# david-wb/tiny-diffusion

Measured on AMD Instinct MI355X. Metric: train images/s (q_sample+fwd+MSE+bwd+allreduce+Adam), MNIST 28x28 UNet fp32; 1000-step sample latency in `sample`, higher is better.
Workload: dtype f32; 1 GPU; diffusion.py unconditional MNIST 28x28 UNet, fp32, train step, batch 256/GPU (BASELINE.json configs[1]); global_batch=256, per_gpu_batch=256, parallelism=dp1

## Files before the change

include/tdx.h:

```cpp
#ifndef TDX_H
#define TDX_H

#include <stddef.h>
#include <stdint.h>

#ifdef __cplusplus
extern "C" {
#endif

#define TDX_VERSION 400

#define TDX_E_BADARG (-1)
#define TDX_E_SHAPE (-2)
#define TDX_E_WORKSPACE (-3)
#define TDX_E_STATE (-4)

typedef void* tdx_stream_t;

int tdx_version(void);
const char* tdx_error_string(int code);


int tdx_q_sample(const float* x0, const float* noise, const int64_t* t,
                 const float* sqrt_ac, const float* sqrt_1mac, float* x_t,
// ... 51 lines not shown

#define TDX_CONV_IN_BNRELU 1
#define TDX_CONV_OUT_BNRELU 2
#define TDX_CONV_OUT_STATS 4

size_t tdx_edge_conv_wgrad_scratch_floats(int B, int H, int W);
int tdx_initial_conv_forward(const float* x, const float* w, const float* bias, float* out, int B, int H, int W,
                             int cin, int cout, tdx_stream_t stream);
int tdx_initial_conv_backward(const float* x, const float* g_out, float* dw, float* db, float* scratch, int B,
                              int H, int W, int cin, int cout, tdx_stream_t stream);
int tdx_initial_conv_input_grad(const float* g_out, const float* w, float* g_x, int B, int H, int W, int cin,
                                int cout, tdx_stream_t stream);
int tdx_final_conv_forward(const float* in, const float* w, const float* bias, float* out, int B, int H, int W,
                           int cout, tdx_stream_t stream);
int tdx_final_conv_backward(const float* in, const float* g_out, const float* w, float* g_in, float* dw, float* db,
                            float* scratch, int B, int H, int W, int cout, tdx_stream_t stream);

int tdx_conv3x3_fwd(const float* in, const float* wpk, const float* bias, float* out,
                    int B, int H, int W, int cin, int cout, int flags,
                    const float* in_scale, const float* in_shift,
                    const float* out_scale, const float* out_shift,
                    float* stats_partial, tdx_stream_t stream);
int tdx_conv3x3_fwd_splitk(const float* in, const float* wpk, const float* bias, float* out,
                           int B, int H, int W, int cin, int cout, int flags,
                           const float* in_scale, const float* in_shift,
                           const float* out_scale, const float* out_shift,
                           float* scratch, size_t scratch_floats, tdx_stream_t stream);
size_t tdx_conv3x3_splitk_scratch_floats(int B, int H, int W, int cin, int cout);
int tdx_conv3x3_wino_ok(int B, int H, int W, int cin, int cout);
int tdx_pack_conv3x3_wino(const float* w_oihw, float* u_fwd, float* u_dgrad, int cout, int cin, tdx_stream_t stream);
int tdx_conv3x3_fwd_wino(const float* in, const float* u, const float* bias, float* out, int B, int H, int W,
                         int cin, int cout, int flags, const float* out_scale, const float* out_shift,
                         float* stats_partial, tdx_stream_t stream);
int tdx_conv3x3_fwd_wino_infer(const float* in, const float* u, const float* bias, float* out, int B, int H, int W,
                               int cin, int cout, const float* out_scale, const float* out_shift, float* scratch,
                               size_t scratch_floats, tdx_stream_t stream);
int tdx_conv3x3_train_algo(int B, int H, int W, int cin, int cout, int role);
int tdx_conv3x3_infer_algo(int B, int H, int W, int cin, int cout);
int tdx_conv3x3_wgrad_wino_splits(int B, int H, int W, int cin, int cout);
int tdx_conv3x3_wgrad_wino(const float* in, const float* dy, float* dw_slabs, int B, int H, int W, int cin, int cout,
                           tdx_stream_t stream);
int tdx_conv3x3_wino_stat_tiles(int B, int H, int W);
int tdx_conv3x3_wino_stat_tile_rows(int B, int H, int W);
int tdx_pack_conv3x3_tiled(const float* w_oihw, float* w_tiled, int cout, int cin, tdx_stream_t stream);
int tdx_conv3x3_fwd_infer(const float* in, const float* w_tiled, const float* bias, float* out, int B, int H, int W,
                          int cin, int cout, const float* out_scale, const float* out_shift, float* scratch,
                          size_t scratch_floats, tdx_stream_t stream);
size_t tdx_conv3x3_infer_scratch_floats(int B, int H, int W, int cin, int cout);
int tdx_conv3x3_fwd_train(const float* in, const float* wpk, const float* bias, float* out, int B, int H, int W,
                          int cin, int cout, int flags, float* stats_partial, float* scratch,
                          size_t scratch_floats, tdx_stream_t stream);
size_t tdx_conv3x3_train_scratch_floats(int B, int H, int W, int cin, int cout);
int tdx_conv3x3_stat_tiles(int B, int H, int W, int cin, int cout);
int tdx_conv3x3_stat_tile_rows(int B, int H, int W, int cin, int cout);
int tdx_conv3x3_shape_ok(int B, int H, int W, int cin, int cout);
int tdx_conv3x3_tile_shape(int B, int H, int W, int cin, int cout, int role);

int tdx_conv3x3_dgrad(const float* dy, const float* w_dgrad, float* dx, int B, int H, int W,
                      int cin, int cout, tdx_stream_t stream);

int tdx_conv3x3_wgrad_splits(int B, int H, int W, int cin, int cout);
int tdx_conv3x3_wgrad(const float* in, const float* dy, float* dw_slabs,
                      int B, int H, int W, int cin, int cout, int flags,
                      const float* in_scale, const float* in_shift, tdx_stream_t stream);
int tdx_conv3x3_wgrad_reduce(const float* dw_slabs, float* dw_oihw, int splits, int cout, int cin,
                             tdx_stream_t stream);
// ... 178 lines not shown
```

tiny_diffusion_amd/_lib.py:

```python
from __future__ import annotations

import ctypes as C
import os

import torch

from . import _build

_c_float_p = C.c_void_p
_c_i64_p = C.c_void_p
_ptr = C.c_void_p


class TdxError(RuntimeError):
    pass


def _load():
    path = _build.LIB
    if not os.path.exists(path):
        if os.environ.get("TDX_NO_AUTOBUILD"):
            raise TdxError(
                f"{path} not found: build it with `python -m tiny_diffusion_amd._build` "
                "(there is no CPU fallback for the HIP path)"
# ... 16 lines not shown


lib = _load()

_SIGS = {
    "tdx_version": (C.c_int, []),
    "tdx_error_string": (C.c_char_p, [C.c_int]),
    "tdx_q_sample": (C.c_int, [_ptr, _ptr, _ptr, _ptr, _ptr, _ptr, C.c_int, C.c_int, _ptr]),
    "tdx_q_sample_philox": (C.c_int, [_ptr, _ptr, _ptr, _ptr, _ptr, _ptr, C.c_int, C.c_int,
                                      C.c_uint64, C.c_uint64, _ptr]),
    "tdx_p_sample_step": (C.c_int, [_ptr, _ptr, _ptr, _ptr, _ptr, _ptr, C.c_int64, _ptr]),
    "tdx_p_sample_step_philox": (C.c_int, [_ptr, _ptr, _ptr, _ptr, _ptr, C.c_int64, C.c_uint64, _ptr]),
    "tdx_u8_gather_normalize": (C.c_int, [_ptr, _ptr, _ptr, C.c_int, C.c_int, C.c_float, C.c_float, _ptr]),
    "tdx_mse_loss": (C.c_int, [_ptr, _ptr, _ptr, _ptr, C.c_float, C.c_int64, _ptr]),
    "tdx_mse_scratch_bytes": (C.c_size_t, []),
    "tdx_mse_loss_grad": (C.c_int, [_ptr, _ptr, _ptr, _ptr, C.c_float, C.c_int64, _ptr, _ptr]),
    "tdx_adam_step": (C.c_int, [_ptr, _ptr, _ptr, _ptr, C.c_int64, C.c_float, C.c_float, C.c_float,
                                C.c_float, C.c_int, C.c_float, _ptr]),
    "tdx_adam_clip_scratch_bytes": (C.c_size_t, []),
    "tdx_adam_step_clip": (C.c_int, [_ptr, _ptr, _ptr, _ptr, C.c_int64, C.c_float, C.c_float, C.c_float, C.c_float,
                                     C.c_int, C.c_float, C.c_float, _ptr, _ptr, _ptr]),
    "tdx_edge_conv_wgrad_scratch_floats": (C.c_size_t, [C.c_int] * 3),
    "tdx_initial_conv_forward": (C.c_int, [_ptr, _ptr, _ptr, _ptr, C.c_int, C.c_int, C.c_int, C.c_int, C.c_int, _ptr]),
    "tdx_initial_conv_backward": (C.c_int, [_ptr, _ptr, _ptr, _ptr, _ptr, C.c_int, C.c_int, C.c_int, C.c_int, C.c_int,
                                            _ptr]),
    "tdx_final_conv_forward": (C.c_int, [_ptr, _ptr, _ptr, _ptr, C.c_int, C.c_int, C.c_int, C.c_int, _ptr]),
    "tdx_final_conv_backward": (C.c_int, [_ptr, _ptr, _ptr, _ptr, _ptr, _ptr, _ptr, C.c_int, C.c_int, C.c_int, C.c_int,
                                          _ptr]),
    "tdx_pack_conv3x3": (C.c_int, [_ptr, _ptr, _ptr, C.c_int, C.c_int, _ptr]),
    "tdx_conv3x3_wino_ok": (C.c_int, [C.c_int] * 5),
    "tdx_pack_conv3x3_wino": (C.c_int, [_ptr, _ptr, _ptr, C.c_int, C.c_int, _ptr]),
    "tdx_conv3x3_fwd_wino": (C.c_int, [_ptr, _ptr, _ptr, _ptr, C.c_int, C.c_int, C.c_int, C.c_int, C.c_int, C.c_int, _ptr,
                                       _ptr, _ptr, _ptr]),
    "tdx_conv3x3_fwd_wino_infer": (C.c_int, [_ptr, _ptr, _ptr, _ptr, C.c_int, C.c_int, C.c_int, C.c_int, C.c_int, _ptr, _ptr,
                                             _ptr, C.c_size_t, _ptr]),
    "tdx_conv3x3_train_algo": (C.c_int, [C.c_int] * 6),
    "tdx_conv3x3_infer_algo": (C.c_int, [C.c_int] * 5),
    "tdx_conv3x3_wgrad_wino_splits": (C.c_int, [C.c_int] * 5),
    "tdx_conv3x3_wgrad_wino": (C.c_int, [_ptr, _ptr, _ptr, C.c_int, C.c_int, C.c_int, C.c_int, C.c_int, _ptr]),
    "tdx_conv3x3_wino_stat_tiles": (C.c_int, [C.c_int] * 3),
    "tdx_conv3x3_wino_stat_tile_rows": (C.c_int, [C.c_int] * 3),
    "tdx_pack_conv3x3_tiled": (C.c_int, [_ptr, _ptr, C.c_int, C.c_int, _ptr]),
    "tdx_conv3x3_fwd_infer": (C.c_int, [_ptr, _ptr, _ptr, _ptr, C.c_int, C.c_int, C.c_int, C.c_int, C.c_int, _ptr, _ptr,
                                        _ptr, C.c_size_t, _ptr]),
    "tdx_conv3x3_infer_scratch_floats": (C.c_size_t, [C.c_int] * 5),
    "tdx_conv3x3_fwd": (C.c_int, [_ptr, _ptr, _ptr, _ptr, C.c_int, C.c_int, C.c_int, C.c_int, C.c_int,
                                  C.c_int, _ptr, _ptr, _ptr, _ptr, _ptr, _ptr]),
    "tdx_conv3x3_fwd_splitk": (C.c_int, [_ptr, _ptr, _ptr, _ptr, C.c_int, C.c_int, C.c_int, C.c_int, C.c_int,
                                         C.c_int, _ptr, _ptr, _ptr, _ptr, _ptr, C.c_size_t, _ptr]),
    "tdx_conv3x3_splitk_scratch_floats": (C.c_size_t, [C.c_int] * 5),
    "tdx_conv3x3_fwd_train": (C.c_int, [_ptr, _ptr, _ptr, _ptr, C.c_int, C.c_int, C.c_int, C.c_int, C.c_int, C.c_int,
                                        _ptr, _ptr, C.c_size_t, _ptr]),
    "tdx_conv3x3_train_scratch_floats": (C.c_size_t, [C.c_int] * 5),
    "tdx_conv3x3_stat_tiles": (C.c_int, [C.c_int] * 5),
    "tdx_conv3x3_stat_tile_rows": (C.c_int, [C.c_int] * 5),
    "tdx_conv3x3_wgrad_splits": (C.c_int, [C.c_int] * 5),
    "tdx_diag_conv_occupancy": (C.c_int, [C.c_int]),
    "tdx_conv3x3_wgrad_splits_bf16": (C.c_int, [C.c_int] * 5),
    "tdx_conv3x3_fwd_bf16_io": (C.c_int, [_ptr] * 4 + [C.c_int] * 6 + [_ptr] * 5 + [C.c_int, _ptr]),
    "tdx_conv3x3_wgrad_bf16_io": (C.c_int, [_ptr] * 3 + [C.c_int] * 6 + [_ptr] * 2 + [C.c_int, _ptr]),
    "tdx_conv3x3_shape_ok": (C.c_int, [C.c_int] * 5),
    "tdx_conv3x3_tile_shape": (C.c_int, [C.c_int] * 6),
    "tdx_conv3x3_wgrad": (C.c_int, [_ptr, _ptr, _ptr, C.c_int, C.c_int, C.c_int, C.c_int, C.c_int,
                                    C.c_int, _ptr, _ptr, _ptr]),
    "tdx_conv3x3_wgrad_reduce": (C.c_int, [_ptr, _ptr, C.c_int, C.c_int, C.c_int, _ptr]),
    "tdx_bn_finalize": (C.c_int, [_ptr, C.c_int, C.c_int, C.c_int64, C.c_int, _ptr, _ptr, _ptr, _ptr, _ptr,
# ... 126 lines not shown
```

tiny_diffusion_amd/csrc/conv3x3.hip:

```cpp
#include "internal.h"
#include <cstring>
#include <type_traits>

#define BK 32
#define BKP 36

#include "conv_shared.h"

template <int BM, int BN, bool IN_BN, int EPI>
__global__ void __launch_bounds__(256)
conv3x3_igemm_kernel(ConvArgs a) {
  constexpr int WGM = 2, WGN = 2;
  constexpr int WTM = BM / WGM, WTN = BN / WGN;
  constexpr int TM = WTM / 32, TN = WTN / 32;
  constexpr int AI = BM / 32, BI = BN / 32;
  static_assert(TM >= 1 && TN >= 1, "wave tile must hold a 32x32 MFMA tile");

  extern __shared__ __attribute__((aligned(16))) float smem[];
  float* As = smem;
  float* Bs = smem + 2 * BM * BKP;

  const int tid = threadIdx.x;
  const int lane = tid & 63, wave = tid >> 6;
  const int l31 = lane & 31, half = lane >> 5;
// ... 764 lines not shown
  if (!strcmp(key, "sample_fuse")) { g_tdx_sample_fuse = value & 7; return 0; }
  if (!strcmp(key, "sample_defer_max")) { g_tdx_sample_defer_max = value; return 0; }
  if (!strcmp(key, "sample_tables")) { g_tdx_sample_tables = value != 0; return 0; }
  if (!strcmp(key, "sample_halves")) { g_tdx_sample_halves = value != 0; return 0; }
  if (!strcmp(key, "sample_halves_min")) { g_tdx_sample_halves_min = value > 2 ? value : 2; return 0; }
  if (!strcmp(key, "bnbwd_fused")) { g_tdx_bnbwd_fused = value & 7; return 0; }
  if (!strcmp(key, "conv_hybrid")) { g_conv_hybrid = value != 0; return 0; }
  if (!strcmp(key, "splitk_fused")) { g_splitk_fused = value != 0; return 0; }
  if (!strcmp(key, "splitk_train")) { g_splitk_train = value != 0; return 0; }
  if (!strcmp(key, "splitk_train_t64")) { g_splitk_train_t64 = value > 0 ? value : 1024; return 0; }
  if (!strcmp(key, "splitk_train_target")) { g_splitk_train_target = value > 0 ? value : 1536; return 0; }
  if (!strcmp(key, "splitk_train_any")) { g_splitk_train_any = value != 0; return 0; }
  if (!strcmp(key, "time_proj_early")) { g_tdx_time_proj_early = value != 0; return 0; }
  if (!strcmp(key, "time_stage_diag")) { g_tdx_time_stage = value == 6 ? 6 : 14; return 0; }
  if (!strcmp(key, "time_l1_impl")) { g_tdx_time_l1_impl = value; return 0; }
  if (!strcmp(key, "input_copy")) { g_tdx_input_copy = value; return 0; }
  if (!strcmp(key, "conv_dbg")) { g_conv_dbg = value; return 0; }
  if (!strcmp(key, "bf16_materialize")) { g_tdx_bf16_materialize = value ? 1 : 0; return 0; }
  if (!strcmp(key, "bf16_thin")) { g_tdx_bf16_thin = value < 0 ? 0 : value; return 0; }
  if (!strcmp(key, "bf16_ring")) { g_tdx_bf16_ring = value ? 1 : 0; return 0; }
  if (!strcmp(key, "bf16_wgrad9")) { g_tdx_wgrad9 = value ? 1 : 0; return 0; }
  if (!strcmp(key, "bf16_wgrad_swz")) { g_tdx_wgrad_bf16s = value ? 1 : 0; return 0; }
  if (!strcmp(key, "conv_stamp")) { g_conv_stamp = value; g_tdx_probe_stamp = value; return 0; }
  if (!strcmp(key, "wgrad_small")) { g_wgrad_small = value; return 0; }
  if (!strcmp(key, "wino")) { g_tdx_wino = value != 0; return 0; }
  if (!strcmp(key, "wino_infer")) { g_tdx_wino_infer = value != 0; return 0; }
  if (!strcmp(key, "wino_infer_min_units")) { g_tdx_wino_infer_min_units = value >= 0 ? value : 700; return 0; }
  if (!strcmp(key, "wino_infer_ovh")) { g_wino_infer_ovh = value >= 0 ? value : 2; return 0; }
  if (!strcmp(key, "wino_infer_red")) { g_wino_infer_red = value >= 0 ? value : 3; return 0; }
  if (!strcmp(key, "wino_wgrad")) { g_tdx_wino_wgrad = value != 0; return 0; }
  if (!strcmp(key, "wino_wgrad_min_tiles")) { g_tdx_wino_wgrad_min_tiles = value > 0 ? value : 1024; return 0; }
  if (!strcmp(key, "wino_wgrad_target")) { g_tdx_wino_wgrad_target = value > 0 ? value : 512; return 0; }
  if (!strcmp(key, "wino_min_wgs")) { g_tdx_wino_min_wgs = value > 0 ? value : 1; return 0; }
  if (!strcmp(key, "wino_rows")) { g_tdx_wino_rows = value != 0; return 0; }
  if (!strcmp(key, "wino_rows_min_stages")) { g_tdx_wino_rows_min_stages = value > 0 ? value : 16; return 0; }
  if (!strcmp(key, "infer_ring")) { g_tdx_infer_ring = value != 0; return 0; }
  if (!strcmp(key, "infer_stages")) { g_infer_stages = value == 3 ? 3 : 4; return 0; }
  if (!strcmp(key, "infer_splits")) { g_infer_splits = value > 0 ? value : 0; return 0; }
  if (!strcmp(key, "infer_ovh")) { g_infer_ovh = value >= 0 ? value : 4; return 0; }
  if (!strcmp(key, "infer_red")) { g_infer_red = value >= 0 ? value : 12; return 0; }
  if (!strcmp(key, "infer_cus")) { g_tdx_infer_cus = value > 0 && value <= 256 ? value : 256; return 0; }
  if (!strcmp(key, "wgrad9_wgs")) { g_wgrad9_wgs = value > 0 ? value : 0; return 0; }
  if (!strcmp(key, "wgrad_plan")) { g_wgrad_plan = value; return 0; }
  if (!strcmp(key, "wgrad_rounds")) { g_wgrad_rounds = value; return 0; }
  if (!strcmp(key, "conv_dma")) { g_conv_dma = value; return 0; }
  if (!strcmp(key, "wgrad_target")) { g_wgrad_target = value > 0 ? value : 2048; return 0; }
  if (!strcmp(key, "wgrad_target_big")) { g_wgrad_target_big = value > 0 ? value : 0; return 0; }
  return TDX_E_BADARG;
}

static TileCfg pick_tile(int64_t M, int cout) {
  const TileCfg cands[3] = {{128, 128}, {128, 64}, {64, 64}};
  if (g_force_tile >= 1 && g_force_tile <= 3 && cout % cands[g_force_tile - 1].bn == 0)
    return cands[g_force_tile - 1];
  for (int i = 0; i < 3; ++i) {
    if (cout % cands[i].bn) continue;
    if (i == 2) return cands[i];
    const int64_t tiles = ((M + cands[i].bm - 1) / cands[i].bm) * (cout / cands[i].bn);
    if (tiles < g_min_tiles) continue;
    const int64_t rounds = (tiles + 255) / 256;
    if ((double)(rounds * 256) <= 1.035 * (double)tiles) return cands[i];
  }
  return cands[2];
}

template <int BM, int BN>
// ... 1179 lines not shown
```

tiny_diffusion_amd/csrc/conv3x3_wino.hip:

```cpp
#include "internal.h"
#include "conv_shared.h"

extern unsigned* g_tdx_diag_buffer;
extern size_t g_tdx_diag_bytes;
extern int g_tdx_probe_stamp;

constexpr int WT = 64;
constexpr int WN = 64;
constexpr int WK = 8;
constexpr int A_ST = 16 * WT * WK;
constexpr int B_ST = 16 * WN * WK;
constexpr int STAGE = A_ST + B_ST;

struct WinoArgs {
  const float* in;
  const float* u;
  const float* bias;
  float* out;
  const float* out_scale;
  const float* out_shift;
  float* stats;
  int B, H, W, Cin, Cout, th, tw, NT, tilesN, M;
  float rcp_tpi, rcp_tw;
  int per;
  int compact;
  unsigned long long* stamps;
};

constexpr int OLD = 68;
constexpr int TAB_OFF = 2 * STAGE;
typedef unsigned u32x4 __attribute__((ext_vector_type(4)));

template <int EPI, int XH = -1>
__device__ __forceinline__ void wino_epilogue(const WinoArgs& a, float* out, const float* bias, f32x16 (&acc)[16], float* smem,
                                              int tblk, int n0, int wm, int wn, int l31, int half, int tid,
                                              const f32x4* xin = nullptr) {
#if defined(__HIP_DEVICE_COMPILE__)
  const unsigned* tab = reinterpret_cast<const unsigned*>(smem + TAB_OFF);
  const int cl = wn * 32 + l31, col = n0 + cl;
  const float bv = bias ? bias[col] : 0.f;
  float osc = 1.f, osh = 0.f;
  if (EPI == EPI_BNRELU) { osc = a.out_scale[col]; osh = a.out_shift[col]; }
  float csum = 0.f, cnt = 0.f;
  float* ot = smem;
  f32x4 pv[8];
#pragma unroll
  for (int r = 0; r < 16; ++r) {
    if (XH >= 0 && (r & 3) == 0) {
#pragma unroll
      for (int p = 0; p < 8; ++p) pv[p] = xin[(p * 4 + (r >> 2)) * 64];
    }
    auto M = [&](int p) { return XH >= 0 && (p >> 3) != XH ? pv[p & 7][r & 3] : acc[p][r]; };
    float s0[4], s1[4];
#pragma unroll
    for (int nu = 0; nu < 4; ++nu) {
      s0[nu] = M(0 + nu) + M(4 + nu) + M(8 + nu);
      s1[nu] = M(4 + nu) - M(8 + nu) - M(12 + nu);
    }
    float y[4] = {s0[0] + s0[1] + s0[2], s0[1] - s0[2] - s0[3], s1[0] + s1[1] + s1[2], s1[1] - s1[2] - s1[3]};
    const int tl = wm * 32 + (r & 3) + 8 * (r >> 2) + 4 * half;
    const unsigned m = tab[2 * tl + 1];
#pragma unroll
    for (int q = 0; q < 4; ++q) {
      float val = y[q] + bv;
      if (EPI == EPI_BNRELU) val = fmaxf(fmaf(val, osc, osh), 0.f);
      const bool ok = (m >> q) & 1u;
      if (XH < 0) ot[(tl * 4 + q) * OLD + cl] = val;
      csum += ok ? val : 0.f;
      cnt += ok ? 1.f : 0.f;
      y[q] = ok ? val : 0.f;
    }
    acc[0][r] = y[0]; acc[1][r] = y[1]; acc[4][r] = y[2]; acc[5][r] = y[3];
    acc[2][r] = (m & 1u) ? 1.f : 0.f;
    acc[3][r] = (m & 2u) ? 1.f : 0.f;
    acc[6][r] = (m & 4u) ? 1.f : 0.f;
    acc[7][r] = (m & 8u) ? 1.f : 0.f;
  }
  if (XH >= 0) {
    __syncthreads();
#pragma unroll
    for (int r = 0; r < 16; ++r) {
      const int tl = wm * 32 + (r & 3) + 8 * (r >> 2) + 4 * half;
      ot[(tl * 4 + 0) * OLD + cl] = acc[0][r]; ot[(tl * 4 + 1) * OLD + cl] = acc[1][r];
      ot[(tl * 4 + 2) * OLD + cl] = acc[4][r]; ot[(tl * 4 + 3) * OLD + cl] = acc[5][r];
    }
  }
  __syncthreads();
  {
    const auto rsrc_out = __builtin_amdgcn_make_buffer_rsrc(out, 0, (int)((int64_t)a.M * a.Cout * 4), 0x00020000);
    const int c4 = (tid & 15) * 4, q = (tid >> 4) & 3;
    const unsigned qoff = (unsigned)((((q >> 1) * a.W + (q & 1)) * a.Cout + n0 + c4) * 4);
    const uint2* tab2 = reinterpret_cast<const uint2*>(tab);
    const float* src = ot + (tid >> 4) * OLD + c4;
#pragma unroll
    for (int i = 0; i < 16; ++i) {
      const uint2 e = tab2[4 * i + (tid >> 6)];
      const unsigned off = ((e.y >> q) & 1u) ? e.x + qoff : 0x80000000u;
      const f32x4 v = *reinterpret_cast<const f32x4*>(src + i * 16 * OLD);
      __builtin_amdgcn_raw_buffer_store_b128(__builtin_bit_cast(u32x4, v), rsrc_out, off, 0, 0);
    }
  }
  if (EPI == EPI_STATS) {
    float* red = smem + 256 * OLD;
    const float s = csum + __shfl_xor(csum, 32, 64);
    const float n = cnt + __shfl_xor(cnt, 32, 64);
    if (half == 0) { red[wm * 64 + cl] = s; red[128 + wm * 64 + cl] = n; }
    __syncthreads();
    if (tid < 64) {
      const float ts = red[tid] + red[64 + tid];
      const float tn = red[128 + tid] + red[192 + tid];
      red[256 + tid] = tn > 0.f ? ts / tn : 0.f;
      a.stats[((size_t)tblk * 2 + 0) * a.Cout + n0 + tid] = ts;
    }
    __syncthreads();
    const float mean = red[256 + cl];
    float q = 0.f;
#pragma unroll
    for (int r = 0; r < 16; ++r) {
      const float d0 = acc[0][r] - mean, d1 = acc[1][r] - mean, d2 = acc[4][r] - mean, d3 = acc[5][r] - mean;
      q = fmaf(d0 * acc[2][r], d0, q); q = fmaf(d1 * acc[3][r], d1, q);
      q = fmaf(d2 * acc[6][r], d2, q); q = fmaf(d3 * acc[7][r], d3, q);
    }
    q += __shfl_xor(q, 32, 64);
    __syncthreads();
    if (half == 0) red[wm * 64 + cl] = q;
    __syncthreads();
    if (tid < 64) a.stats[((size_t)tblk * 2 + 1) * a.Cout + n0 + tid] = red[tid] + red[64 + tid];
  }
#endif
}

#if defined(__HIP_DEVICE_COMPILE__)
// ... 333 lines not shown
    gg[3][c] = g[6 + c];
  }
#pragma unroll
  for (int r = 0; r < 4; ++r) {
    U[r * 4 + 0] = gg[r][0];
    U[r * 4 + 1] = 0.5f * (gg[r][0] + gg[r][1] + gg[r][2]);
    U[r * 4 + 2] = 0.5f * (gg[r][0] - gg[r][1] + gg[r][2]);
    U[r * 4 + 3] = gg[r][2];
  }
  if (b.uf[u]) {
    float* dst = b.uf[u] + (((size_t)cb * nkb + kb) * 16) * 512 + cl * 8 + k8;
#pragma unroll
    for (int p = 0; p < 16; ++p) dst[p * 512] = U[p];
  }
  if (b.ud[u]) {
    float* dst = b.ud[u] + (((size_t)(ci >> 6) * (cout / 8) + (co >> 3)) * 16) * 512 + (ci & 63) * 8 + (co & 7);
    constexpr int ps = 512;
#pragma unroll
    for (int p = 0; p < 16; ++p) {
      const int xi = p >> 2, nu = p & 3;
      const int sx = xi == 0 ? 3 : xi == 3 ? 0 : xi, sn = nu == 0 ? 3 : nu == 3 ? 0 : nu;
      dst[p * ps] = U[sx * 4 + sn];
    }
  }
}

static int wino_tile_rows(int H, int W) {
  const int th = (H + 1) / 2, tw = (W + 1) / 2;
  if (!(H & 1) && !(W & 1)) return 4 * WT;
  if (WT % (th * tw) == 0) return (WT / (th * tw)) * H * W;
  return 0;
}

extern "C" int tdx_conv3x3_wino_ok(int B, int H, int W, int cin, int cout) {
  if (B <= 0 || H <= 0 || W <= 0 || cin <= 0 || cout <= 0 || cin % WK || cout % WN) return 0;
  if (!wino_tile_rows(H, W)) return 0;
  const int64_t M = (int64_t)B * H * W;
  return M * cin * 4 < (1ll << 31) && M * cout * 4 < (1ll << 31) && (int64_t)cout * 16 * cin * 4 < (1ll << 31) &&
         (int64_t)B * ((H + 1) / 2) * ((W + 1) / 2) + 64 < (1ll << 24);
}

extern "C" int tdx_conv3x3_wino_stat_tile_rows(int B, int H, int W) { (void)B; return wino_tile_rows(H, W); }
extern "C" int tdx_conv3x3_wino_stat_tiles(int B, int H, int W) {
  const int th = (H + 1) / 2, tw = (W + 1) / 2;
  return cdiv((int64_t)B * th * tw, WT);
}

int tdx_pack_conv3x3_wino_pad(const float* w_oihw, float* u_fwd, float* u_dgrad, int cout, int cin_real, int cin,
                              tdx_stream_t stream);

int tdx_pack_conv3x3_wino_batch(TdxWinoPackBatch* b, tdx_stream_t stream) {
  if (!b || b->count <= 0 || b->count > TDX_PACK_MAX) return TDX_E_BADARG;
  int blocks = 0;
  for (int u = 0; u < b->count; ++u) {
    if (!b->w[u] || b->cin_real[u] <= 0 || b->cin_real[u] > b->cin[u] || b->cin[u] % 64 || b->cout[u] % 64) return TDX_E_BADARG;
    b->start[u] = blocks;
    blocks += (b->cin[u] / 8) * (b->cout[u] / 64);
  }
  pack_wino_batch_kernel<<<blocks, 512, 0, to_stream(stream)>>>(*b);
  TDX_CHECK_LAUNCH();
  return 0;
}

int tdx_pack_conv3x3_wino_pad(const float* w_oihw, float* u_fwd, float* u_dgrad, int cout, int cin_real, int cin,
                              tdx_stream_t stream) {
  if (!w_oihw || cout <= 0 || cin <= 0 || cin_real <= 0 || cin_real > cin) return TDX_E_BADARG;
  if (cin % 64 || cout % 64) return TDX_E_SHAPE;
  if (!u_fwd && !u_dgrad) return 0;
  TdxWinoPackBatch b{};
  b.count = 1;
  b.w[0] = w_oihw; b.uf[0] = u_fwd; b.ud[0] = u_dgrad; b.cout[0] = cout; b.cin[0] = cin; b.cin_real[0] = cin_real;
  return tdx_pack_conv3x3_wino_batch(&b, stream);
}

extern "C" int tdx_pack_conv3x3_wino(const float* w_oihw, float* u_fwd, float* u_dgrad, int cout, int cin,
                                     tdx_stream_t stream) {
  return tdx_pack_conv3x3_wino_pad(w_oihw, u_fwd, u_dgrad, cout, cin, cin, stream);
}

int g_tdx_wino_rows = 1;
int g_tdx_wino_rows_min_stages = 16;

int tdx_conv3x3_wino_launch(const float* in, const float* u, const float* bias, float* out, int B, int H, int W,
                            int cin, int cout, int flags, const float* out_scale, const float* out_shift,
                            float* stats_partial, int splits, int per, tdx_stream_t stream) {
  if (!in || !u || !out) return TDX_E_BADARG;
  if (!tdx_conv3x3_wino_ok(B, H, W, cin, cout)) return TDX_E_SHAPE;
  if (flags & ~(TDX_CONV_OUT_BNRELU | TDX_CONV_OUT_STATS)) return TDX_E_BADARG;
  if ((flags & TDX_CONV_OUT_BNRELU) && (!out_scale || !out_shift)) return TDX_E_BADARG;
  if ((flags & TDX_CONV_OUT_STATS) && (!stats_partial || (flags & TDX_CONV_OUT_BNRELU))) return TDX_E_BADARG;
  if (splits < 1 || (splits > 1 && (per < 1 || (int64_t)per * (splits - 1) >= cin / WK))) return TDX_E_BADARG;
  WinoArgs a{};
  a.in = in; a.u = u; a.bias = bias; a.out = out; a.out_scale = out_scale; a.out_shift = out_shift;
  a.stats = stats_partial;
  a.B = B; a.H = H; a.W = W; a.Cin = cin; a.Cout = cout;
  a.th = (H + 1) / 2; a.tw = (W + 1) / 2;
  a.NT = B * a.th * a.tw;
  a.rcp_tpi = 1.0f / (float)(a.th * a.tw); a.rcp_tw = 1.0f / (float)a.tw;
  a.tilesN = cout / WN;
  a.M = B * H * W;
  a.per = per;
  a.compact = cdiv(a.NT, WT) < 64;
  const dim3 grid(a.compact ? cdiv(a.NT, WT) * a.tilesN : (cdiv(a.NT, WT) + 7) / 8 * 8 * a.tilesN, splits);
  a.stamps = g_tdx_probe_stamp == 3 && g_tdx_diag_buffer && (size_t)grid.x * grid.y * 64 <= g_tdx_diag_bytes
                 ? reinterpret_cast<unsigned long long*>(g_tdx_diag_buffer) : nullptr;
  const size_t lds = (size_t)2 * STAGE * sizeof(float) + WT * 2 * sizeof(unsigned);
  hipStream_t st = to_stream(stream);
#define TDX_WINO_LAUNCH(EPI_, SPL_, ROWS_)                                                                       \
  do {                                                                                                           \
    auto kern = conv3x3_wino_kernel<EPI_, SPL_, ROWS_>;                                                          \
    static bool attr_set = false;                                                                                \
    if (!attr_set) {                                                                                             \
      hipError_t e = hipFuncSetAttribute(reinterpret_cast<const void*>(kern),                                    \
                                         hipFuncAttributeMaxDynamicSharedMemorySize, (int)lds);                  \
      if (e != hipSuccess) return (int)e;                                                                        \
      attr_set = true;                                                                                           \
    }                                                                                                            \
    kern<<<grid, 256, lds, st>>>(a);                                                                             \
  } while (0)
  const bool rows = g_tdx_wino_rows && cin / WK >= g_tdx_wino_rows_min_stages;
  if (splits > 1) TDX_WINO_LAUNCH(EPI_PLAIN, true, false);
  else if (flags & TDX_CONV_OUT_BNRELU) TDX_WINO_LAUNCH(EPI_BNRELU, false, false);
  else if (flags & TDX_CONV_OUT_STATS) {
    if (rows) TDX_WINO_LAUNCH(EPI_STATS, false, true);
    else TDX_WINO_LAUNCH(EPI_STATS, false, false);
  } else if (rows) TDX_WINO_LAUNCH(EPI_PLAIN, false, true);
  else TDX_WINO_LAUNCH(EPI_PLAIN, false, false);
#undef TDX_WINO_LAUNCH
  TDX_CHECK_LAUNCH();
  return 0;
}

extern "C" int tdx_conv3x3_fwd_wino(const float* in, const float* u, const float* bias, float* out, int B, int H, int W,
                                    int cin, int cout, int flags, const float* out_scale, const float* out_shift,
                                    float* stats_partial, tdx_stream_t stream) {
  return tdx_conv3x3_wino_launch(in, u, bias, out, B, H, W, cin, cout, flags, out_scale, out_shift, stats_partial, 1, 0,
                                 stream);
}

constexpr int GT8 = 8;
constexpr int XS_F = GT8 * 16 * 64;
constexpr int ES_F = GT8 * 4 * 64;
constexpr int WST_F = XS_F + ES_F;
constexpr int WNST = 3;
constexpr int WG_MAX_CHUNK = 1024;
constexpr int WG_XCH_F = 4 * 8 * 16 * 64;
constexpr size_t WG_LDS = 131072;
static_assert((size_t)WNST * WST_F * 4 + (size_t)WG_MAX_CHUNK * 4 <= WG_LDS && (size_t)WG_XCH_F * 4 <= WG_LDS, "LDS");

struct WinoWgArgs {
  const float* in;
  const float* dy;
  float* slabs;
  int B, H, W, Cin, Cout, th, tw, NT, M;
  int tilesCo, tilesCi, chunk;
  unsigned long long* stamps;
};

#if defined(__HIP_DEVICE_COMPILE__)
__device__ __forceinline__ unsigned long long wg_lanes16(unsigned m) {
  const unsigned lo = ((m & 1u) ? 0x0000ffffu : 0u) | ((m & 2u) ? 0xffff0000u : 0u);
  const unsigned hi = ((m & 4u) ? 0x0000ffffu : 0u) | ((m & 8u) ? 0xffff0000u : 0u);
  return (unsigned long long)hi << 32 | lo;
}
__device__ __forceinline__ unsigned wg_sel(unsigned long long mask, unsigned x, unsigned y) {
  unsigned r;
  asm("v_cndmask_b32_e64 %0, %1, %2, %3" : "=v"(r) : "v"(y), "v"(x), "s"(mask));
  return r;
}
#endif
// ... 311 lines not shown
```

tiny_diffusion_amd/csrc/internal.h:

```cpp
#pragma once
#include "common.h"

int tdx_copy_floats(const float* src, float* dst, size_t n, hipStream_t st);
int tdx_copy_segments(const float* const* src, float* const* dst, const size_t* n, int count, hipStream_t st);
int tdx_pixel_sum(const void* g, float* out, int B, int HW, int C, hipStream_t st, int io16 = 0);
int tdx_reduce_partials(const float* partial, float* out, int nblk, int stride, int count,
                        hipStream_t st);
int tdx_initial_conv_fwd(const float* x, const float* w, const float* bias, void* out, int B, int H,
                         int W, int cin, int cout_real, hipStream_t st, int io16 = 0);
int tdx_small_conv_wgrad_blocks(int B, int H, int W);
int tdx_small_conv_partial_width(void);
int tdx_initial_conv_wgrad(const float* x, const void* g, float* partial, float* dw, float* db,
                           int B, int H, int W, int cin, int cout_real, hipStream_t st, int io16 = 0);
int tdx_initial_conv_dgrad(const void* g_x0, const float* w, float* g_x, int B, int H, int W, int cin,
                           int cout_real, hipStream_t st, int io16 = 0);
int tdx_final_conv_fwd(const void* in, const float* w, const float* bias, float* out, int B, int H,
                       int W, int cout, hipStream_t st, int io16 = 0);
int tdx_final_conv_fwd_psample(const void* in, const float* w, const float* bias, float* eps_out, int B, int H, int W,
                               int cout, float* x, const float* z, const float* coef, const int32_t* t_idx,
                               uint64_t seed, int philox, int64_t* counter_dec, hipStream_t st, int io16 = 0,
                               int64_t elem0 = 0, const int64_t* tau = nullptr);
int tdx_final_conv_dgrad(const float* g_out, const float* w, void* g_in, int B, int H, int W,
                         int cout, hipStream_t st, int io16 = 0);
int tdx_final_conv_wgrad(const void* in, const float* g_out, float* partial, float* dw, float* db,
// ... 13 lines not shown
int tdx_conv3x3_fwd_splitk_fused(const float* in, const float* wpk, const float* bias, float* out, int B, int H,
                                 int W, int cin, int cout, int flags, const float* out_scale,
                                 const float* out_shift, float* scratch, size_t scratch_floats, unsigned* counters,
                                 int n_counters, tdx_stream_t stream, TdxSplitDefer* defer = nullptr,
                                 TdxPoolFuse* pool = nullptr);
int tdx_conv3x3_fwd_infer_ex(const float* in, const float* w_tiled, const float* bias, float* out, int B, int H, int W,
                             int cin, int cout, const float* out_scale, const float* out_shift, float* scratch,
                             size_t scratch_floats, tdx_stream_t stream, TdxSplitDefer* defer, TdxPoolFuse* pool);
extern int g_tdx_infer_ring;
extern int g_tdx_infer_cus;
#define TDX_PACK_MAX 13
struct TdxPackBatch {
  const float* w[TDX_PACK_MAX];
  float* wf[TDX_PACK_MAX];
  float* wd[TDX_PACK_MAX];
  int cout[TDX_PACK_MAX], cin[TDX_PACK_MAX], cin_real[TDX_PACK_MAX], chunk_start[TDX_PACK_MAX];
  int count;
};
int tdx_pack_conv3x3_batch(TdxPackBatch* b, tdx_stream_t stream);
struct TdxWinoPackBatch {
  const float* w[TDX_PACK_MAX];
  float* uf[TDX_PACK_MAX];
  float* ud[TDX_PACK_MAX];
  int cout[TDX_PACK_MAX], cin[TDX_PACK_MAX], cin_real[TDX_PACK_MAX], start[TDX_PACK_MAX];
  int count;
};
int tdx_pack_conv3x3_wino_batch(TdxWinoPackBatch* b, tdx_stream_t stream);
extern "C" int tdx_conv3x3_wino_ok(int B, int H, int W, int cin, int cout);
extern "C" int tdx_conv3x3_wino_stat_tiles(int B, int H, int W);
extern "C" int tdx_conv3x3_wino_stat_tile_rows(int B, int H, int W);
extern int g_tdx_wino, g_tdx_wino_min_wgs;
extern int g_tdx_wino_wgrad, g_tdx_wino_wgrad_min_tiles, g_tdx_wino_wgrad_target;
extern int g_tdx_wino_rows, g_tdx_wino_rows_min_stages;
extern "C" int tdx_conv3x3_wgrad_wino_splits(int B, int H, int W, int cin, int cout);
extern "C" int tdx_conv3x3_wgrad_wino(const float* in, const float* dy, float* dw_slabs, int B, int H, int W, int cin, int cout,
                                      tdx_stream_t stream);
extern int g_tdx_wino_infer_min_units;
extern int g_tdx_wino_infer;
int tdx_conv3x3_wino_launch(const float* in, const float* u, const float* bias, float* out, int B, int H, int W,
                            int cin, int cout, int flags, const float* out_scale, const float* out_shift,
                            float* stats_partial, int splits, int per, tdx_stream_t stream);
int tdx_conv3x3_fwd_wino_infer_ex(const float* in, const float* u, const float* bias, float* out, int B, int H, int W,
                                  int cin, int cout, const float* out_scale, const float* out_shift, float* scratch,
                                  size_t scratch_floats, tdx_stream_t stream, TdxSplitDefer* defer, TdxPoolFuse* pool);
int tdx_pack_conv3x3_tiled_batch(TdxPackBatch* b, tdx_stream_t stream);
int tdx_pack_conv3x3_tiled_pad(const float* w_oihw, float* w_tiled, int cout, int cin_real, int cin, tdx_stream_t stream);
int tdx_pack_conv3x3_batch_bf16(TdxPackBatch* b, tdx_stream_t stream);
int tdx_pack_conv3x3_pad(const float* w_oihw, float* w_fwd, float* w_dgrad, int cout, int cin_real,
                         int cin, tdx_stream_t stream);
int tdx_conv3x3_wgrad_reduce_pad(const float* dw_slabs, float* dw_oihw, int splits, int cout, int cin,
                                 int cin_real, tdx_stream_t stream);
int tdx_time_embed_bwd_ex(const float* tf, const int64_t* y, const float* const* P, float* const* G,
                          const float* pre, const float* emb, const float* const* gk, const int* ldg,
                          const int* widths, float* scratch, int B, int ncls, hipStream_t st,
                          const int64_t* t_i64 = nullptr, int td = 0, int parts = 7);
int tdx_bn_moments(const float* stats_partial, int tiles, int tile_rows, int64_t count, int C, double* mom,
                   hipStream_t st);
int tdx_bn_finalize_moments(const double* mom, int C, const float* gamma, const float* beta, float* running_mean,
                            float* running_var, int64_t* nbt, float* scale, float* shift, float* save_mean,
                            float* save_rstd, hipStream_t st);
int tdx_bn_relu_bwd_sync(float* g, const float* y, int64_t rows, int C, const float* scale, const float* shift,
                         const float* save_mean, const float* save_rstd, const float* gamma, float* dgamma,
                         float* dbeta, float* dbias, float* scratch, int training, tdx_allreduce_fn sync,
                         void* sync_user, double* mom, tdx_stream_t stream, int io16 = 0);
extern int g_tdx_time_l1_impl;
extern int g_tdx_input_copy;
// ... 67 lines not shown
```

tiny_diffusion_amd/csrc/unet.hip:

```cpp
#include "internal.h"
#include <algorithm>
#include <cstdlib>
#include <mutex>
#include <new>
#include <string>
#include <vector>

namespace {

struct UnitDef {
  int cin, cout, hw;
  int in_bn;
  int cin_real;
};

struct NetSpec {
  int in_ch, hw0, out_hw;
  int x0_ch, x0_real;
  int overlap;
  int time_dim;
  int enc_hw[4];
  int dec_hw[3];
  int skip_ch[3];
  UnitDef units[13];
// ... 898 lines not shown
      TDX_HIP(hipStreamWaitEvent(u->side, u->ev_dy[i], 0));
    }
    if (i + 2 < 13 && u->red_pending[i + 2]) {
      TDX_HIP(hipStreamWaitEvent(wst, u->ev_red[i + 2], 0));
      u->red_pending[i + 2] = false;
    }
    if (bf16)
      RC(tdx_conv3x3_wgrad_bf16_io(in, g, slab, B, d.hw, d.hw, d.cin, d.cout, bn_on_load ? TDX_CONV_IN_BNRELU : 0, isc,
                                   ish, io16, reinterpret_cast<tdx_stream_t>(wst)));
    else if (u->wino_w[i] && !bn_on_load)
      RC(tdx_conv3x3_wgrad_wino(in, g, slab, B, d.hw, d.hw, d.cin, d.cout, reinterpret_cast<tdx_stream_t>(wst)));
    else
      RC(tdx_conv3x3_wgrad(in, g, slab, B, d.hw, d.hw, d.cin, d.cout, bn_on_load ? TDX_CONV_IN_BNRELU : 0, isc, ish,
                           reinterpret_cast<tdx_stream_t>(wst)));
    TDX_HIP(hipEventRecord(u->ev_w[i], wst));
    if (red_st != wst) TDX_HIP(hipStreamWaitEvent(red_st, u->ev_w[i], 0));
    RC(tdx_conv3x3_wgrad_reduce_pad(slab, G[TDX_P_UNIT0 + 4 * i],
                                    bf16 ? tdx_conv3x3_wgrad_splits_bf16(B, d.hw, d.hw, d.cin, d.cout)
                                    : u->wino_w[i] && !bn_on_load ? tdx_conv3x3_wgrad_wino_splits(B, d.hw, d.hw, d.cin, d.cout)
                                                                  : tdx_conv3x3_wgrad_splits(B, d.hw, d.hw, d.cin, d.cout),
                                    d.cout, d.cin, d.cin_real, reinterpret_cast<tdx_stream_t>(red_st)));
    if (red_st != wst) {
      TDX_HIP(hipEventRecord(u->ev_red[i], red_st));
      u->red_pending[i] = true;
    }
    GBuf* gbuf = find(g);
    gbuf->w_unit = i;
    gbuf->age = ++clock;
    float* g_in;
    RC(acquire(g, nullptr, &g_in));
    if (bf16)
      RC(tdx_conv3x3_fwd_bf16_io(g, u->wpack + u->wd_off[i], nullptr, g_in, B, d.hw, d.hw, d.cout, d.cin, 0, nullptr,
                                 nullptr, nullptr, nullptr, nullptr, io16, stream));
    else if (u->wino_d[i])
      RC(tdx_conv3x3_fwd_wino(g, u->upack + u->ud_off[i], nullptr, g_in, B, d.hw, d.hw, d.cout, d.cin, 0, nullptr, nullptr,
                              nullptr, stream));
    else if (d.in_bn) {
      const float* pss = ws + L.ss[i - 1];
      int nblk = 0;
      RC(tdx_conv3x3_dgrad_bnbwd(g, u->wpack + u->wd_off[i], g_in, B, d.hw, d.hw, d.cout, d.cin, ws + L.Y[i - 1], pss,
                                 pss + d.cin, pss + 2 * d.cin, pss + 3 * d.cin, ws + L.bnscr, &nblk, ws + L.ksplit,
                                 L.ksplit_floats, stream));
      if (nblk > 0) { u->bw_unit = i - 1; u->bw_nblk = nblk; }
    } else
      RC(tdx_conv3x3_fwd_train(g, u->wpack + u->wd_off[i], nullptr, g_in, B, d.hw, d.hw, d.cout, d.cin, 0, nullptr,
                               ws + L.ksplit, L.ksplit_floats, stream));
    *g_in_out = g_in;
    return 0;
  };
  auto bw_y = [&](int i) -> const float* { return ws + L.Y[i]; };
  auto plain_unit_bwd = [&](int i, const float* in) -> int {
    float* g_in;
    RC(unit_bwd(i, in, &g_in));
    g_next = g_in;
    return 0;
  };
  auto ssc = [&](int i) { return ws + L.ss[i]; };
  auto ssh = [&](int i) { return ws + L.ss[i] + S.units[i].cout; };
  auto time_path_parts = [&](int parts) -> int {
    return tdx_time_embed_bwd(u->kind, reinterpret_cast<const int64_t*>(ws + L.t),
                              u->num_classes > 0 ? reinterpret_cast<const int64_t*>(ws + L.y) : nullptr,
                              P, G, ws + L.sin, ws + L.pre, ws + L.emb, ws + L.gtp[0], ws + L.gtp[1],
                              ws + L.gtp[2], ws + L.timescr, B, u->num_classes, u->side2, S.time_dim, parts);
  };
  auto dec_level_bwd = [&](int k) -> int {
    const int ua = 7 + 2 * k;
    const int prev = k == 0 ? 6 : 6 + 2 * k;
// ... 289 lines not shown
```

Measured before the change: 27160 images/s.

## Fuse BN-backward partial sums into Winograd dgrad epilogue

Adds a Winograd dgrad epilogue that, while storing the input gradient, also loads the saved pre-BN activation and accumulates the per-channel BN-backward reductions (masked by ReLU) into block partials. The UNet backward then uses this fused Winograd dgrad for BN-input units that previously ran plain Winograd dgrad followed by a separate BN-backward reduction pass. It also relaxes the shape check for non-stats launches so more shapes can use Winograd. The aim is to remove a full extra read of the gradient tensor and a kernel launch, at the cost of higher register pressure (16 prefetched vectors) and extra shared memory traffic in the epilogue. Arguments reach the kernel through thread-local global state.

```diff
diff --git a/include/tdx.h b/include/tdx.h
--- a/include/tdx.h
+++ b/include/tdx.h
@@ -107,6 +107,9 @@
 int tdx_conv3x3_fwd_wino(const float* in, const float* u, const float* bias, float* out, int B, int H, int W,
                          int cin, int cout, int flags, const float* out_scale, const float* out_shift,
                          float* stats_partial, tdx_stream_t stream);
+int tdx_conv3x3_dgrad_wino_bnbwd(const float* in, const float* u, float* out, int B, int H, int W, int cin, int cout,
+                                 const float* y, const float* scale, const float* shift, const float* mean,
+                                 const float* rstd, float* partial, int* nblk, tdx_stream_t stream);
 int tdx_conv3x3_fwd_wino_infer(const float* in, const float* u, const float* bias, float* out, int B, int H, int W,
                                int cin, int cout, const float* out_scale, const float* out_shift, float* scratch,
                                size_t scratch_floats, tdx_stream_t stream);
diff --git a/tiny_diffusion_amd/_lib.py b/tiny_diffusion_amd/_lib.py
--- a/tiny_diffusion_amd/_lib.py
+++ b/tiny_diffusion_amd/_lib.py
@@ -72,6 +72,7 @@
     "tdx_pack_conv3x3_wino": (C.c_int, [_ptr, _ptr, _ptr, C.c_int, C.c_int, _ptr]),
     "tdx_conv3x3_fwd_wino": (C.c_int, [_ptr, _ptr, _ptr, _ptr, C.c_int, C.c_int, C.c_int, C.c_int, C.c_int, C.c_int, _ptr,
                                        _ptr, _ptr, _ptr]),
+    "tdx_conv3x3_dgrad_wino_bnbwd": (C.c_int, [_ptr, _ptr, _ptr] + [C.c_int] * 5 + [_ptr] * 6 + [C.POINTER(C.c_int), _ptr]),
     "tdx_conv3x3_fwd_wino_infer": (C.c_int, [_ptr, _ptr, _ptr, _ptr, C.c_int, C.c_int, C.c_int, C.c_int, C.c_int, _ptr, _ptr,
                                              _ptr, C.c_size_t, _ptr]),
     "tdx_conv3x3_train_algo": (C.c_int, [C.c_int] * 6),
diff --git a/tiny_diffusion_amd/csrc/conv3x3.hip b/tiny_diffusion_amd/csrc/conv3x3.hip
--- a/tiny_diffusion_amd/csrc/conv3x3.hip
+++ b/tiny_diffusion_amd/csrc/conv3x3.hip
@@ -820,6 +820,7 @@
   if (!strcmp(key, "wino_wgrad_min_tiles")) { g_tdx_wino_wgrad_min_tiles = value > 0 ? value : 1024; return 0; }
   if (!strcmp(key, "wino_wgrad_target")) { g_tdx_wino_wgrad_target = value > 0 ? value : 512; return 0; }
   if (!strcmp(key, "wino_min_wgs")) { g_tdx_wino_min_wgs = value > 0 ? value : 1; return 0; }
+  if (!strcmp(key, "wino_bnbwd")) { g_tdx_wino_bnbwd = value != 0; return 0; }
   if (!strcmp(key, "wino_rows")) { g_tdx_wino_rows = value != 0; return 0; }
   if (!strcmp(key, "wino_rows_min_stages")) { g_tdx_wino_rows_min_stages = value > 0 ? value : 16; return 0; }
   if (!strcmp(key, "infer_ring")) { g_tdx_infer_ring = value != 0; return 0; }
diff --git a/tiny_diffusion_amd/csrc/conv3x3_wino.hip b/tiny_diffusion_amd/csrc/conv3x3_wino.hip
--- a/tiny_diffusion_amd/csrc/conv3x3_wino.hip
+++ b/tiny_diffusion_amd/csrc/conv3x3_wino.hip
@@ -25,9 +25,13 @@
   int per;
   int compact;
   unsigned long long* stamps;
+  const float* bw_y;
+  const float* bw_scale; const float* bw_shift; const float* bw_mean; const float* bw_rstd;
+  float* bw_partial;
 };
 
 constexpr int OLD = 68;
+static_assert(256 * OLD + 16 * 2 * 64 <= 2 * STAGE, "EPI_BNBWD: the lane groups' sums fit behind the output image");
 constexpr int TAB_OFF = 2 * STAGE;
 typedef unsigned u32x4 __attribute__((ext_vector_type(4)));
 
@@ -43,6 +47,20 @@
   if (EPI == EPI_BNRELU) { osc = a.out_scale[col]; osh = a.out_shift[col]; }
   float csum = 0.f, cnt = 0.f;
   float* ot = smem;
+  f32x4 bw_yv[16];
+  auto bw_request = [&]() {
+    const auto rsrc_y = __builtin_amdgcn_make_buffer_rsrc(const_cast<float*>(a.bw_y), 0, (int)((int64_t)a.M * a.Cout * 4), 0x00020000);
+    const int c4 = (tid & 15) * 4, q = (tid >> 4) & 3;
+    const unsigned qoff = (unsigned)((((q >> 1) * a.W + (q & 1)) * a.Cout + n0 + c4) * 4);
+    const uint2* tab2 = reinterpret_cast<const uint2*>(tab);
+#pragma unroll
+    for (int i = 0; i < 16; ++i) {
+      const uint2 e = tab2[4 * i + (tid >> 6)];
+      const unsigned off = ((e.y >> q) & 1u) ? e.x + qoff : 0x80000000u;
+      bw_yv[i] = __builtin_bit_cast(f32x4, __builtin_amdgcn_raw_buffer_load_b128(rsrc_y, off, 0, 0));
+    }
+  };
+  if (EPI == EPI_BNBWD && XH >= 0) bw_request();
   f32x4 pv[8];
 #pragma unroll
   for (int r = 0; r < 16; ++r) {
@@ -85,6 +103,7 @@
       ot[(tl * 4 + 2) * OLD + cl] = acc[4][r]; ot[(tl * 4 + 3) * OLD + cl] = acc[5][r];
     }
   }
+  if (EPI == EPI_BNBWD && XH < 0) bw_request();
   __syncthreads();
   {
     const auto rsrc_out = __builtin_amdgcn_make_buffer_rsrc(out, 0, (int)((int64_t)a.M * a.Cout * 4), 0x00020000);
@@ -92,12 +111,40 @@
     const unsigned qoff = (unsigned)((((q >> 1) * a.W + (q & 1)) * a.Cout + n0 + c4) * 4);
     const uint2* tab2 = reinterpret_cast<const uint2*>(tab);
     const float* src = ot + (tid >> 4) * OLD + c4;
+    f32x4 bsc, bsh, bmu, brs, bs1 = {0.f, 0.f, 0.f, 0.f}, bs2 = {0.f, 0.f, 0.f, 0.f};
+    if (EPI == EPI_BNBWD) {
+      bsc = *reinterpret_cast<const f32x4*>(a.bw_scale + n0 + c4); bsh = *reinterpret_cast<const f32x4*>(a.bw_shift + n0 + c4);
+      bmu = *reinterpret_cast<const f32x4*>(a.bw_mean + n0 + c4); brs = *reinterpret_cast<const f32x4*>(a.bw_rstd + n0 + c4);
+    }
 #pragma unroll
     for (int i = 0; i < 16; ++i) {
       const uint2 e = tab2[4 * i + (tid >> 6)];
       const unsigned off = ((e.y >> q) & 1u) ? e.x + qoff : 0x80000000u;
       const f32x4 v = *reinterpret_cast<const f32x4*>(src + i * 16 * OLD);
       __builtin_amdgcn_raw_buffer_store_b128(__builtin_bit_cast(u32x4, v), rsrc_out, off, 0, 0);
+      if (EPI == EPI_BNBWD) {
+        const bool ok = (e.y >> q) & 1u;
+#pragma unroll
+        for (int k = 0; k < 4; ++k) {
+          const float yk = bw_yv[i][k];
+          const float gz = ok && fmaf(yk, bsc[k], bsh[k]) > 0.f ? v[k] : 0.f;
+          bs1[k] += gz;
+          bs2[k] += gz * ((yk - bmu[k]) * brs[k]);
+        }
+      }
+    }
+    if (EPI == EPI_BNBWD) {
+      float* red = smem + 256 * OLD;
+      *reinterpret_cast<f32x4*>(red + ((tid >> 4) * 2 + 0) * 64 + c4) = bs1;
+      *reinterpret_cast<f32x4*>(red + ((tid >> 4) * 2 + 1) * 64 + c4) = bs2;
+      __syncthreads();
+      if (tid < 128) {
+        const int sq = tid >> 6, c = tid & 63;
+        float s = 0.f;
+#pragma unroll
+        for (int g = 0; g < 16; ++g) s += red[(g * 2 + sq) * 64 + c];
+        a.bw_partial[((size_t)tblk * 2 + sq) * a.Cout + n0 + c] = s;
+      }
     }
   }
   if (EPI == EPI_STATS) {
@@ -497,13 +544,15 @@
   return 0;
 }
 
-extern "C" int tdx_conv3x3_wino_ok(int B, int H, int W, int cin, int cout) {
+static int wino_shape_ok(int B, int H, int W, int cin, int cout, bool uniform) {
   if (B <= 0 || H <= 0 || W <= 0 || cin <= 0 || cout <= 0 || cin % WK || cout % WN) return 0;
-  if (!wino_tile_rows(H, W)) return 0;
+  if (uniform && !wino_tile_rows(H, W)) return 0;
   const int64_t M = (int64_t)B * H * W;
   return M * cin * 4 < (1ll << 31) && M * cout * 4 < (1ll << 31) && (int64_t)cout * 16 * cin * 4 < (1ll << 31) &&
          (int64_t)B * ((H + 1) / 2) * ((W + 1) / 2) + 64 < (1ll << 24);
 }
+
+extern "C" int tdx_conv3x3_wino_ok(int B, int H, int W, int cin, int cout) { return wino_shape_ok(B, H, W, cin, cout, true); }
 
 extern "C" int tdx_conv3x3_wino_stat_tile_rows(int B, int H, int W) { (void)B; return wino_tile_rows(H, W); }
 extern "C" int tdx_conv3x3_wino_stat_tiles(int B, int H, int W) {
@@ -544,20 +593,27 @@
 }
 
 int g_tdx_wino_rows = 1;
+int g_tdx_wino_bnbwd = 1;
+struct WinoBw { const float *y, *scale, *shift, *mean, *rstd; float* partial; };
+static thread_local WinoBw g_wino_bw = {};
 int g_tdx_wino_rows_min_stages = 16;
 
 int tdx_conv3x3_wino_launch(const float* in, const float* u, const float* bias, float* out, int B, int H, int W,
                             int cin, int cout, int flags, const float* out_scale, const float* out_shift,
                             float* stats_partial, int splits, int per, tdx_stream_t stream) {
   if (!in || !u || !out) return TDX_E_BADARG;
-  if (!tdx_conv3x3_wino_ok(B, H, W, cin, cout)) return TDX_E_SHAPE;
   if (flags & ~(TDX_CONV_OUT_BNRELU | TDX_CONV_OUT_STATS)) return TDX_E_BADARG;
+  if (!wino_shape_ok(B, H, W, cin, cout, flags & TDX_CONV_OUT_STATS)) return TDX_E_SHAPE;
+  const bool bw = g_wino_bw.partial != nullptr;
+  if (bw && (flags || splits != 1)) return TDX_E_BADARG;
   if ((flags & TDX_CONV_OUT_BNRELU) && (!out_scale || !out_shift)) return TDX_E_BADARG;
   if ((flags & TDX_CONV_OUT_STATS) && (!stats_partial || (flags & TDX_CONV_OUT_BNRELU))) return TDX_E_BADARG;
   if (splits < 1 || (splits > 1 && (per < 1 || (int64_t)per * (splits - 1) >= cin / WK))) return TDX_E_BADARG;
   WinoArgs a{};
   a.in = in; a.u = u; a.bias = bias; a.out = out; a.out_scale = out_scale; a.out_shift = out_shift;
   a.stats = stats_partial;
+  a.bw_y = g_wino_bw.y; a.bw_scale = g_wino_bw.scale; a.bw_shift = g_wino_bw.shift; a.bw_mean = g_wino_bw.mean;
+  a.bw_rstd = g_wino_bw.rstd; a.bw_partial = g_wino_bw.partial;
   a.B = B; a.H = H; a.W = W; a.Cin = cin; a.Cout = cout;
   a.th = (H + 1) / 2; a.tw = (W + 1) / 2;
   a.NT = B * a.th * a.tw;
@@ -589,6 +645,9 @@
   else if (flags & TDX_CONV_OUT_STATS) {
     if (rows) TDX_WINO_LAUNCH(EPI_STATS, false, true);
     else TDX_WINO_LAUNCH(EPI_STATS, false, false);
+  } else if (bw) {
+    if (rows) TDX_WINO_LAUNCH(EPI_BNBWD, false, true);
+    else TDX_WINO_LAUNCH(EPI_BNBWD, false, false);
   } else if (rows) TDX_WINO_LAUNCH(EPI_PLAIN, false, true);
   else TDX_WINO_LAUNCH(EPI_PLAIN, false, false);
 #undef TDX_WINO_LAUNCH
@@ -601,6 +660,25 @@
                                     float* stats_partial, tdx_stream_t stream) {
   return tdx_conv3x3_wino_launch(in, u, bias, out, B, H, W, cin, cout, flags, out_scale, out_shift, stats_partial, 1, 0,
                                  stream);
+}
+
+extern "C" int tdx_conv3x3_dgrad_wino_bnbwd(const float* in, const float* u, float* out, int B, int H, int W, int cin,
+                                            int cout, const float* y, const float* scale, const float* shift,
+                                            const float* mean, const float* rstd, float* partial, int* nblk,
+                                            tdx_stream_t stream) {
+  if (!nblk) return TDX_E_BADARG;
+  *nblk = 0;
+  const int64_t blocks = cdiv((int64_t)B * ((H + 1) / 2) * ((W + 1) / 2), WT);
+  const bool fits = blocks <= cdiv((int64_t)B * H * W, 64);
+  if (!g_tdx_wino_bnbwd || !y || !partial || !fits || !wino_shape_ok(B, H, W, cin, cout, false))
+    return tdx_conv3x3_wino_launch(in, u, nullptr, out, B, H, W, cin, cout, 0, nullptr, nullptr, nullptr, 1, 0, stream);
+  if (!scale || !shift || !mean || !rstd) return TDX_E_BADARG;
+  g_wino_bw = {y, scale, shift, mean, rstd, partial};
+  const int rc = tdx_conv3x3_wino_launch(in, u, nullptr, out, B, H, W, cin, cout, 0, nullptr, nullptr, nullptr, 1, 0, stream);
+  g_wino_bw = {};
+  if (rc) return rc;
+  *nblk = (int)blocks;
+  return 0;
 }
 
 constexpr int GT8 = 8;
diff --git a/tiny_diffusion_amd/csrc/internal.h b/tiny_diffusion_amd/csrc/internal.h
--- a/tiny_diffusion_amd/csrc/internal.h
+++ b/tiny_diffusion_amd/csrc/internal.h
@@ -69,6 +69,11 @@
 extern int g_tdx_wino, g_tdx_wino_min_wgs;
 extern int g_tdx_wino_wgrad, g_tdx_wino_wgrad_min_tiles, g_tdx_wino_wgrad_target;
 extern int g_tdx_wino_rows, g_tdx_wino_rows_min_stages;
+extern int g_tdx_wino_bnbwd;
+extern "C" int tdx_conv3x3_dgrad_wino_bnbwd(const float* in, const float* u, float* out, int B, int H, int W, int cin,
+                                            int cout, const float* y, const float* scale, const float* shift,
+                                            const float* mean, const float* rstd, float* partial, int* nblk,
+                                            tdx_stream_t stream);
 extern "C" int tdx_conv3x3_wgrad_wino_splits(int B, int H, int W, int cin, int cout);
 extern "C" int tdx_conv3x3_wgrad_wino(const float* in, const float* dy, float* dw_slabs, int B, int H, int W, int cin, int cout,
                                       tdx_stream_t stream);
diff --git a/tiny_diffusion_amd/csrc/unet.hip b/tiny_diffusion_amd/csrc/unet.hip
--- a/tiny_diffusion_amd/csrc/unet.hip
+++ b/tiny_diffusion_amd/csrc/unet.hip
@@ -954,7 +954,13 @@
     if (bf16)
       RC(tdx_conv3x3_fwd_bf16_io(g, u->wpack + u->wd_off[i], nullptr, g_in, B, d.hw, d.hw, d.cout, d.cin, 0, nullptr,
                                  nullptr, nullptr, nullptr, nullptr, io16, stream));
-    else if (u->wino_d[i])
+    else if (u->wino_d[i] && d.in_bn && g_tdx_wino_bnbwd) {
+      const float* pss = ws + L.ss[i - 1];
+      int nblk = 0;
+      RC(tdx_conv3x3_dgrad_wino_bnbwd(g, u->upack + u->ud_off[i], g_in, B, d.hw, d.hw, d.cout, d.cin, ws + L.Y[i - 1], pss,
+                                      pss + d.cin, pss + 2 * d.cin, pss + 3 * d.cin, ws + L.bnscr, &nblk, stream));
+      if (nblk > 0) { u->bw_unit = i - 1; u->bw_nblk = nblk; }
+    } else if (u->wino_d[i])
       RC(tdx_conv3x3_fwd_wino(g, u->upack + u->ud_off[i], nullptr, g_in, B, d.hw, d.hw, d.cout, d.cin, 0, nullptr, nullptr,
                               nullptr, stream));
     else if (d.in_bn) {
```

Measured after the change: 27370 images/s (median of 6 runs). About the same (+0.8%).
